# Streampunk/phaneron

Measured on AMD Instinct MI355X. Metric: frames/sec, 4-layer 2160p50 composite pipeline (v210 unpack->CSC->combine->CSC->v210 pack), higher is better.
Workload: dtype f32

## Files before the change

phaneron_amd/csrc/ph_api.cpp:

```cpp
#include <algorithm>
#include <atomic>
#include <chrono>
#include <cstdarg>
#include <cstdio>
#include <cstring>
#include <dlfcn.h>
#include <map>
#include <mutex>
#include <string>
#include <vector>

#include "../../include/phaneron_hip.h"
#include "ph_fused_field.h"
#include "ph_internal.h"
#include "ph_kernels.h"
#include "ph_lut_host.h"

using ph::KernelId;
using namespace ph;

namespace {
thread_local std::string g_err;
}

// ... 792 lines not shown
    ctx->luts.erase(it);
  }
  if (blob) {
    for (int q = 0; q < 3; ++q) hipStreamSynchronize(ctx->streams[q]);
    hipFree(blob);
  }
  return PH_OK;
}

int ph_lut_register(ph_ctx *ctx, const void *dev, const float *host) {
  if (!ctx || !dev || !host) return fail(PH_E_INVALID, "ph_lut_register: NULL argument");
  int rc = set_device(ctx);
  if (rc) return rc;
  ph_lut_unregister(ctx, dev);
  std::vector<uint32_t> blob;
  ph::LutHostInfo info;
  LutEntry e;
  if (ph::lut_compress(host, ph::kLutMaxLdsBytes, blob, info)) {
    if (!ctx->lds_base_checked.load()) {
      uint32_t *probe = nullptr, base = ~0u;
      PH_HIP(hipMalloc(&probe, 4));
      hipError_t pe = ph::launch_lds_base_probe(ctx->streams[0], probe);
      if (pe == hipSuccess) pe = hipStreamSynchronize(ctx->streams[0]);
      if (pe == hipSuccess) pe = hipMemcpy(&base, probe, 4, hipMemcpyDeviceToHost);
      hipFree(probe);
      if (pe != hipSuccess) return fail(PH_E_HIP, "ph_lut_register: LDS base probe: %s", hipGetErrorString(pe));
      if (base != 0) return fail(PH_E_HIP, "ph_lut_register: dynamic shared memory starts at LDS address %u, not 0: the table kernels cannot run", base);
      ctx->lds_base_checked.store(true);
    }
    const size_t blob_bytes = blob.size() * sizeof(uint32_t);
    PH_HIP(hipMalloc(&e.blob_dev, blob_bytes));
    PH_HIP(hipMemcpy(e.blob_dev, blob.data(), blob_bytes, hipMemcpyHostToDevice));
    e.view = ph::lut_view(info, e.blob_dev);
  }
  {
    std::lock_guard<std::mutex> lock(ctx->mu);
    ctx->luts[dev] = e;
  }
  return e.view.bytes ? 1 : 0;
}

int ph_lut_layout_of(const float *host, ph_lut_layout *layout, void *lds_image, size_t capacity) {
  if (!host || !layout) return fail(PH_E_INVALID, "ph_lut_layout_of: NULL argument");
  std::vector<uint32_t> blob;
  ph::LutHostInfo info;
  memset(layout, 0, sizeof(*layout));
  if (!ph::lut_compress(host, ph::kLutMaxLdsBytes, blob, info)) return 0;
  const ph::LutView v = ph::lut_view(info, nullptr);
  layout->lds_bytes = info.bytes, layout->hole = info.hole, layout->delta_off = info.delta_off, layout->shift = info.shift;
  layout->index_bias = (uint32_t)info.bias, layout->a_scale = v.a_scale;
  if (lds_image) {
    if (capacity < info.bytes) return fail(PH_E_INVALID, "ph_lut_layout_of: the image needs %u bytes, %zu given", info.bytes, capacity);
    memset(lds_image, 0, info.hole);
    memcpy(static_cast<char *>(lds_image) + info.hole, blob.data(), info.bytes - info.hole);
  }
  return (int)info.bytes;
}

int ph_debug_fused_lut_k(const float *host, uint32_t k5[5]) {
  if (!host || !k5) return fail(PH_E_INVALID, "ph_debug_fused_lut_k: NULL argument");
  std::vector<uint32_t> blob;
  ph::LutHostInfo info;
  if (!ph::lut_compress(host, ph::kLutMaxLdsBytes, blob, info)) return 0;
  const ph::FusedLutK k = ph::fused_lut_k(ph::lut_view(info, nullptr));
  memcpy(k5, &k, 5 * sizeof(uint32_t));
  return (int)info.bytes;
}
uint32_t ph_debug_fused_job_of(uint32_t wg_per_job, uint32_t block) {
  return wg_per_job ? ph::fused_job_of(block, ph::fused_wg_magic(wg_per_job)) : 0;
}
int ph_debug_fused_field_quad(uint32_t width, uint32_t height, int interlace, uint32_t g, uint32_t *f, uint32_t *line, uint32_t *col) {
  if (!width || width % 48) return fail(PH_E_INVALID, "ph_debug_fused_field_quad: width %u (the field launches take width %% 48 == 0)", width);
  if (interlace != 1 && interlace != 3) return fail(PH_E_INVALID, "ph_debug_fused_field_quad: interlace %d (a field: 1 or 3)", interlace);
  const uint32_t qpl = width / 6;
  if ((uint64_t)qpl * height * qpl >= (1ull << 32)) return fail(PH_E_INVALID, "ph_debug_fused_field_quad: %u x %u is beyond the kernels' division by reciprocal", width, height);
  if (g >= qpl * (height / 2u)) return fail(PH_E_INVALID, "ph_debug_fused_field_quad: quad %u is outside the field (%u quads)", g, qpl * (height / 2u));
  const ph::FieldQuad q = ph::fused_field_quad(g, qpl, (uint32_t)(((1ull << 32) + qpl - 1) / qpl), interlace == 3 ? 1u : 0u);
  if (f) *f = q.f;
  if (line) *line = q.line;
  if (col) *col = q.col;
  return PH_OK;
}
int ph_debug_image_nt(ph_ctx *ctx, size_t bytes) {
  if (!ctx) return fail(PH_E_INVALID, "ph_debug_image_nt: ctx is NULL");
  if (int rc = set_device(ctx)) return rc;
  return (int)ph::image_nt(bytes);
}

int ph_lut_query(ph_ctx *ctx, const void *dev, uint32_t *lds_bytes, uint32_t *toe, uint32_t *shift) {
  if (!ctx) return fail(PH_E_INVALID, "ph_lut_query: ctx is NULL");
  std::lock_guard<std::mutex> lock(ctx->mu);
  auto it = ctx->luts.find(dev);
  const bool have = it != ctx->luts.end();
  if (lds_bytes) *lds_bytes = have ? it->second.view.bytes : 0;
  if (toe) *toe = have ? (uint32_t)it->second.view.bias : 0;
  if (shift) *shift = have ? 23 - it->second.view.shift : 0;
  return PH_OK;
}

int ph_ctx_set_option(ph_ctx *ctx, const char *name, int value) {
// ... 29 lines not shown
    if (value != 0 && value != 1) return fail(PH_E_INVALID, "fused_multi_batch: 0 (a launch per such job) or 1 (shared launches)");
    return ctx->fused_multi_batch = value, PH_OK;
  }
  if (0 == strcmp(name, "fused_fields")) {
    if (value != 0 && value != 1) return fail(PH_E_INVALID, "fused_fields: 0 (the plain-layer launches compose the whole frame) or 1 (only the field, where every output takes the same one)");
    return ctx->fused_fields = value, PH_OK;
  }
  if (0 == strcmp(name, "host_pool_mb")) {
    if (value < 0) return fail(PH_E_INVALID, "host_pool_mb: a size in MiB");
    std::vector<ph_ctx::HostBlock> drop;
    {
      std::lock_guard<std::mutex> lock(ctx->mu);
      ctx->host_pool_mb = value;
      ctx->host_peak_bytes = ctx->host_live_bytes;
      while (ctx->host_pooled_bytes > (size_t)value << 20 && !ctx->host_pool.empty()) {
        auto it = std::prev(ctx->host_pool.end());
        ctx->host_pooled_bytes -= it->first;
        drop.push_back(it->second);
        ctx->host_pool.erase(it);
      }
    }
    for (auto &v : drop) {
      hipHostFree(v.p);
      if (v.busy) hipEventDestroy(v.busy);
    }
    return PH_OK;
  }
  return fail(PH_E_INVALID, "unknown option '%s'", name);
}

struct LutRef {
  ph::LutView view{};
  bool found = false;
  const ph::LutView *get() const { return found ? &view : nullptr; }
};
static LutRef lds_view(ph_ctx *ctx, const void *dev) {
  LutRef r;
  if (!ctx || !ctx->use_lds_lut) return r;
  std::lock_guard<std::mutex> lock(ctx->mu);
  auto it = ctx->luts.find(dev);
  if (it == ctx->luts.end() || !it->second.view.bytes) return r;
  r.view = it->second.view, r.found = true;
  return r;
}

extern "C++" void refresh_buf_lut(ph_ctx *ctx, ph_buf *b) {
  if (b->lut_dirty && b->hptr && b->bytes >= 65536 * 4) {
    hipStreamSynchronize(ctx->streams[PH_QUEUE_LOAD]);
    ph_lut_register(ctx, b->dptr, (const float *)b->hptr);
    b->lut_dirty = false;
  }
}

extern "C++" int chan_out_refused(const char *fn, int fmt) {
  return fail(PH_E_INVALID, "%s: the channel kernel does not write %s frames - run the separate kernels: the channel's frame as an image, then the format's writer (ph_pack_write)", fn,
              fmt_name(fmt));
}

extern "C++" bool inject_failure(ph_ctx *ctx) {
  const int v = ctx->fail_launches.load();
  if (v > 0) return true;
  if (v < 0 && ctx->fail_launches.fetch_add(1) == -1) ctx->fail_launches.store(1);
  return false;
}

uint32_t ph_v210_pitch_bytes(uint32_t width) { return width ? ph::v210_pitch_bytes(width) : 0; }

#define PH_LAUNCH(expr)                                                                         \
  do {                                                                                          \
    if (!ctx) return fail(PH_E_INVALID, "%s: ctx is NULL", __func__);                           \
    PH_QUEUE(__func__, queue);                                                                  \
    int rc_ = set_device(ctx);                                                                  \
    if (rc_) return rc_;                                                                        \
    hipError_t e_ = ph::trace_launch(#expr) ? hipSuccess : (expr);                              \
    if (e_ != hipSuccess) return fail(PH_E_HIP, "%s: launch failed: %s", __func__, hipGetErrorString(e_)); \
// ... 44 lines not shown
      PH_LAUNCH(ph::launch_v210_write_lds(stream_of(ctx, queue), in, out, width, height, interlace, cm, *v,
                                          (uint32_t)ctx->props.multiProcessorCount));
  }
  PH_LAUNCH(ph::launch_v210_write(stream_of(ctx, queue), in, out, width, height, interlace, cm, lut));
}

int ph_fused_v210_combine(ph_ctx *ctx, int queue, int n, const void *const *layers, void *out, uint32_t width,
                          uint32_t height, const void *rd_cm, const void *rd_lut, const void *rd_gm,
                          const void *wr_cm, const void *wr_lut) {
  if (n < 1 || n > ph::kMaxLayers) return fail(PH_E_INVALID, "ph_fused_v210_combine: 1..%d layers", ph::kMaxLayers);
  if (!layers || !out || !rd_cm || !rd_lut || !rd_gm || !wr_cm || !wr_lut || !width)
    return fail(PH_E_INVALID, "ph_fused_v210_combine: NULL/zero argument");
  const bool ragged = width % 48 != 0;
  if (width & 1) return fail(PH_E_INVALID, "ph_fused_v210_combine: width %u is odd; run the separate kernels", width);
  if (!height) return PH_OK;
  ph::FusedArgs a{};
  for (int i = 0; i < n; ++i) {
    if (!layers[i]) return fail(PH_E_INVALID, "ph_fused_v210_combine: layer %d is NULL", i);
    a.layers[i] = layers[i];
  }
  a.out = out;
  a.quads_per_line_used = width / 6;
  a.quads_per_line_pitch = ph::v210_pitch_bytes(width) / 16;
  a.total_quads = (ragged ? a.quads_per_line_pitch : a.quads_per_line_used) * height;
  a.tail_px = width % 6, a.magic_qpp = (uint32_t)(((1ull << 32) + a.quads_per_line_pitch - 1) / a.quads_per_line_pitch);
  if (ragged && (uint64_t)a.total_quads * a.quads_per_line_pitch >= (1ull << 32))
    return fail(PH_E_INVALID, "ph_fused_v210_combine: a %u x %u frame with ragged lines is too large; run the separate kernels", width, height);
  a.rd_cm = (const float *)rd_cm, a.rd_lut = (const float *)rd_lut, a.rd_gm = (const float *)rd_gm;
  a.wr_cm = (const float *)wr_cm, a.wr_lut = (const float *)wr_lut;
  if (ctx) {
    const LutRef rref = lds_view(ctx, rd_lut), wref = lds_view(ctx, wr_lut);
    const ph::LutView *rv = rref.get(), *wv = wref.get();
    if (rv && wv) {
      const ph::FusedLdsArgs la = ph::fused_lds_args(a, *rv, *wv);
      PH_LAUNCH(ph::launch_fused_v210_combine_lds(stream_of(ctx, queue), n, la, (uint32_t)ctx->props.multiProcessorCount));
    }
  }
  PH_LAUNCH(ph::launch_fused_v210_combine(stream_of(ctx, queue), n, a));
}

int ph_pack_plane_bytes(int format, uint32_t width, uint32_t height, size_t bytes[3]) {
  if (!bytes || !width) return fail(PH_E_INVALID, "ph_pack_plane_bytes: NULL/zero argument");
  if (const int rc = even_dims("ph_pack_plane_bytes", format, width, height)) return rc;
  const int n = ph::pack_plane_bytes(format, width, height, bytes);
  return n < 0 ? fail(PH_E_INVALID, "ph_pack_plane_bytes: unknown format %d", format) : n;
}

int ph_fused_v210_combine_batch(ph_ctx *ctx, int queue, int jobs, int n, const void *const *layers, void *const *outs,
                                uint32_t width, uint32_t height, const void *rd_cm, const void *rd_lut, const void *rd_gm,
                                const void *wr_cm, const void *wr_lut) {
  if (jobs < 1 || jobs > ph::kMaxBatch) return fail(PH_E_INVALID, "ph_fused_v210_combine_batch: 1..%d jobs", ph::kMaxBatch);
  if (n < 1 || n > ph::kMaxLayers) return fail(PH_E_INVALID, "ph_fused_v210_combine_batch: 1..%d layers", ph::kMaxLayers);
  if (!layers || !outs || !rd_cm || !rd_lut || !rd_gm || !wr_cm || !wr_lut)
    return fail(PH_E_INVALID, "ph_fused_v210_combine_batch: NULL argument");
  for (int j = 0; j < jobs; ++j) {
    if (!outs[j]) return fail(PH_E_INVALID, "ph_fused_v210_combine_batch: output %d is NULL", j);
    for (int l = 0; l < n; ++l)
      if (!layers[j * n + l]) return fail(PH_E_INVALID, "ph_fused_v210_combine_batch: job %d layer %d is NULL", j, l);
  }
  const LutRef rref = lds_view(ctx, rd_lut), wref = lds_view(ctx, wr_lut);
  const ph::LutView *rv = rref.get(), *wv = wref.get();
  if (jobs == 1 || !rv || !wv || !width || width % 48 || !height) {
    for (int j = 0; j < jobs; ++j) {
      int rc = ph_fused_v210_combine(ctx, queue, n, layers + (size_t)j * n, outs[j], width, height, rd_cm, rd_lut, rd_gm,
                                     wr_cm, wr_lut);
      if (rc != PH_OK) return rc;
    }
    return PH_OK;
  }
  ph::FusedArgs f{};
  for (int l = 0; l < n; ++l) f.layers[l] = layers[l];
  f.out = outs[0];
  f.quads_per_line_used = width / 6;
  f.quads_per_line_pitch = ph::v210_pitch_bytes(width) / 16;
  f.total_quads = f.quads_per_line_used * height;
  f.rd_cm = (const float *)rd_cm, f.rd_lut = (const float *)rd_lut, f.rd_gm = (const float *)rd_gm;
  f.wr_cm = (const float *)wr_cm, f.wr_lut = (const float *)wr_lut;
  ph::FusedLdsArgs la = ph::fused_lds_args(f, *rv, *wv);
  la.jobs = (uint32_t)jobs;
  for (int j = 1; j < jobs; ++j) {
    for (int l = 0; l < n; ++l) la.more_layers[j - 1][l] = layers[(size_t)j * n + l];
    la.more_out[j - 1] = outs[j];
  }
  PH_LAUNCH(ph::launch_fused_v210_combine_lds(stream_of(ctx, queue), n, la, (uint32_t)ctx->props.multiProcessorCount));
}

int ph_pack_read(ph_ctx *ctx, int queue, int format, const void *const planes[3], void *out, uint32_t width,
                 uint32_t height, const void *cm, const void *lut, const void *gm) {
  if (!ctx || !planes || !out || !lut || !gm || !width) return fail(PH_E_INVALID, "ph_pack_read: NULL/zero argument");
  if (format == PH_FMT_V210) return ph_v210_read(ctx, queue, planes[0], out, width, height, cm, lut, gm);
  if (const int rc = even_dims("ph_pack_read", format, width, height)) return rc;
  size_t pb[3];
  const int np = ph::pack_plane_bytes(format, width, height, pb);
  if (np < 0) return fail(PH_E_INVALID, "ph_pack_read: unknown format %d", format);
  for (int i = 0; i < np; ++i)
    if (!planes[i]) return fail(PH_E_INVALID, "ph_pack_read: plane %d is NULL", i);
  if (!fmt_rgb8(format) && !cm) return fail(PH_E_INVALID, "ph_pack_read: YCbCr formats need a colMatrix");
  if (!height) return PH_OK;
  PH_LAUNCH(ph::launch_pack_read(stream_of(ctx, queue), format, planes, out, width, height, cm, lut, gm, lds_view(ctx, lut).get(),
                                 (uint32_t)ctx->props.multiProcessorCount));
}

int ph_pack_read_batch(ph_ctx *ctx, int queue, int format, int n, const void *const (*planes)[3], void *const *outs, uint32_t width, uint32_t height,
                       const void *cm, const void *lut, const void *gm) {
  if (!ctx || !planes || !outs || !lut || !gm || !width) return fail(PH_E_INVALID, "ph_pack_read_batch: NULL/zero argument");
  if (n < 1 || n > ph::kMaxLayers) return fail(PH_E_INVALID, "ph_pack_read_batch: 1..%d frames", ph::kMaxLayers);
  if (const int rc = even_dims("ph_pack_read_batch", format, width, height)) return rc;
  const LutRef lref = lds_view(ctx, lut);
  const ph::LutView *v = format == PH_FMT_V210 ? nullptr : lref.get();
  if (n == 1 || !v) {
    if (format == PH_FMT_V210) {
// ... 2126 lines not shown
```

phaneron_amd/csrc/ph_internal.h:

```cpp
#pragma once
#include <atomic>
#include <cstdlib>
#include <map>
#include <mutex>
#include <string>
#include <vector>

#include "../../include/phaneron_hip.h"
#include "ph_kernels.h"
#include "ph_program.h"
#include "ph_spans.h"

static_assert(ph::kSpanLayers == ph::kMaxLayers && ph::kSpanOuts >= ph::kMaxChanOuts && ph::kSpanOuts >= ph::kMaxFusedOuts && ph::kSpanOuts >= ph::kMaxUpOuts,
              "a Footprint holds any job's ranges: ph_spans.h sizes it by these limits without seeing ph_kernels.h");
static_assert(ph::kMaxChanOps <= ph::kSpanLayers * 3, "a channel job's op list is at most three sources per layer");

#pragma GCC visibility push(hidden)
int fail(int code, const char *fmt, ...) __attribute__((format(printf, 2, 3)));
#pragma GCC visibility pop

#define PH_HIP(call)                                                                          \
  do {                                                                                        \
    hipError_t e_ = (call);                                                                   \
    if (e_ != hipSuccess) return fail(PH_E_HIP, "%s failed: %s", #call, hipGetErrorString(e_)); \
  } while (0)

struct LutEntry {
  ph::LutView view{};
  void *blob_dev = nullptr;
};

struct ph_ctx {
  int device = 0;
  std::map<const void *, LutEntry> luts;
  bool use_lds_lut = true;
  int stream_images = 0;
  int stream_threshold_mb = 64;
  hipStream_t streams[3] = {nullptr, nullptr, nullptr};
  hipDeviceProp_t props;
  std::multimap<size_t, void *> pool;
  size_t pooled_bytes = 0, live_buffers = 0, live_bytes = 0;
  struct HostBlock {
    void *p;
    hipEvent_t busy;
    uint64_t seq;
  };
  std::multimap<size_t, HostBlock> host_pool;
  size_t host_pooled_bytes = 0;
  uint64_t host_pool_seq = 0;
  int chan_enlarged = !(getenv("PH_CHAN_ENLARGED") && getenv("PH_CHAN_ENLARGED")[0] == '0');
  int chan_batch_outs = 0;
  int clip_batch = 0;
  int up_v210_tails = 0;
  int fused_multi_wgs = 0;
  int fused_multi_batch = 0;
  int fused_fields = 0;
  std::atomic<int> fail_launches{0};
  int host_pool_mb = 4096;
  size_t host_live_bytes = 0, host_peak_bytes = 0;
  uint64_t host_pins = 0;
  void *chan_index[3] = {nullptr, nullptr, nullptr};
  size_t chan_index_bytes[3] = {0, 0, 0};
// ... 62 lines not shown
```

phaneron_amd/csrc/ph_kernels.h:

```cpp
#pragma once
#include <hip/hip_runtime.h>
#include <stddef.h>
#include <stdint.h>

#include "ph_formats.h"
#include "ph_lut.h"

namespace ph {

constexpr int kMaxLayers = 8;
constexpr int kMaxDynamicLds = 160 * 1024;

extern thread_local uint32_t t_stream_images;
extern thread_local uint32_t t_stream_threshold_mb;
static inline uint32_t image_nt(size_t bytes) {
  return t_stream_images == 2 ? (bytes > ((size_t)t_stream_threshold_mb << 20) ? 1u : 0u) : t_stream_images;
}

struct FusedArgs {
  const void *layers[kMaxLayers];
  void *out;
  uint32_t quads_per_line_used;
  uint32_t quads_per_line_pitch;
  uint32_t total_quads;
// ... 4 lines not shown
constexpr int kMaxBatch = 8;
struct FusedLutK {
  float a_scale, a_base, delta_scale, delta_base;
  uint32_t a_shift;
};
FusedLutK fused_lut_k(const LutView &v);

static inline uint32_t fused_wg_magic(uint32_t wg_per_job) { return (uint32_t)(((1ull << 31) + wg_per_job - 1) / wg_per_job); }
static inline __host__ __device__ uint32_t fused_job_of(uint32_t block, uint32_t magic) {
#if defined(__HIP_DEVICE_COMPILE__)
  return __umulhi(2u * block + 1u, magic);
#else
  return (uint32_t)(((uint64_t)(2u * block + 1u) * magic) >> 32);
#endif
}

struct alignas(64) FusedLdsArgs {
  const uint32_t *rd_blob;
  uint32_t rd_bytes, rd_hole;
  uint32_t total_quads;
  uint32_t wg_per_job;
  uint32_t per_wg;
  uint32_t magic_wg;
  const void *layers[kMaxLayers];
  void *out;
  const float *rd_cm, *rd_gm, *wr_cm;
  FusedLutK rd_k, wr_k;
  uint32_t wr_bytes, wr_hole;
  const uint32_t *wr_blob;
  uint32_t jobs;
  uint32_t quads_per_line_used;
  uint32_t quads_per_line_pitch;
  uint32_t tail_px, magic_qpp;
  const void *more_layers[kMaxBatch - 1][kMaxLayers];
  void *more_out[kMaxBatch - 1];
};
constexpr size_t kFusedHeadBytes = 192;
static_assert(offsetof(FusedLdsArgs, rd_blob) == 0 && offsetof(FusedLdsArgs, rd_bytes) == 8 && offsetof(FusedLdsArgs, rd_hole) == 12 &&
              offsetof(FusedLdsArgs, total_quads) == 16 && offsetof(FusedLdsArgs, wg_per_job) == 20 && offsetof(FusedLdsArgs, per_wg) == 24 &&
              offsetof(FusedLdsArgs, magic_wg) == 28 && offsetof(FusedLdsArgs, layers) == 32,
              "line 0 of the fused kernel's head: ph_kernels_lds.hip reads it by offset");
static_assert(offsetof(FusedLdsArgs, out) == 96 && offsetof(FusedLdsArgs, rd_cm) == 104 && offsetof(FusedLdsArgs, rd_gm) == 112 &&
              offsetof(FusedLdsArgs, wr_cm) == 120, "the head's pointers end with the first 128 bytes");
static_assert(offsetof(FusedLdsArgs, rd_k) == 128 && offsetof(FusedLdsArgs, wr_k) == 148 && offsetof(FusedLdsArgs, wr_bytes) == 168 &&
              offsetof(FusedLdsArgs, wr_hole) == 172 && offsetof(FusedLdsArgs, wr_blob) == 176 && offsetof(FusedLdsArgs, jobs) == 184 &&
              offsetof(FusedLdsArgs, quads_per_line_used) == 188 && offsetof(FusedLdsArgs, quads_per_line_pitch) == kFusedHeadBytes,
              "line 2 of the fused kernel's head");
static_assert(offsetof(FusedLdsArgs, more_layers) >= kFusedHeadBytes, "the batch arrays lie behind the head");
FusedLdsArgs fused_lds_args(const FusedArgs &f, const LutView &rd, const LutView &wr);

constexpr int kMaxFusedOuts = 4;
struct FusedOut {
  uint32_t fmt;
  uint32_t takes;
  uint32_t line_end;
  uint32_t field;
  uint32_t half_pitch;
  uint32_t pad;
  const float *wr_cm;
  void *plane[3];
  LutView wr;
};
struct FusedMultiArgs {
  const void *layers[kMaxLayers];
  uint32_t quads_per_line, total_quads;
  uint32_t magic_qpl, need_line;
  const float *rd_cm, *rd_gm;
  LutView rd;
  uint32_t n_out;
  FusedOut out[kMaxFusedOuts];
};
hipError_t launch_fused_v210_combine_multi(hipStream_t s, int n, const FusedMultiArgs &a, uint32_t num_cus, uint32_t max_wgs);
hipError_t fused_multi_plan(const FusedMultiArgs &a, uint32_t num_cus, uint32_t max_wgs, FusedMultiArgs &b, uint32_t &grid, uint32_t &lds);
struct FusedMultiBatchArgs {
  FusedMultiArgs m;
  const void *layers[kMaxBatch][kMaxLayers];
  void *plane[kMaxBatch][kMaxFusedOuts][3];
};
hipError_t launch_fused_v210_combine_multi_batch(hipStream_t s, int n, uint32_t jobs, const FusedMultiBatchArgs &a, uint32_t num_cus, uint32_t max_wgs);
enum : uint32_t { kFusedCut = 0, kFusedDissolve = 1, kFusedWipeV210 = 2, kFusedWipeF32 = 3 };
struct FusedTransArgs {
  FusedMultiArgs m;
// ... 356 lines not shown
```

phaneron_amd/csrc/ph_kernels_lds.hip:

```cpp
#include "ph_device.h"
#include "ph_kernels.h"
#include "ph_ldslut.h"

#include <atomic>
#include <cstdlib>

#include <type_traits>
#include <utility>

#pragma clang fp contract(off)

#ifndef PH_PROBE
#define PH_PROBE 0
#endif
#if PH_PROBE
constexpr int kProbeWords = 16;
__device__ unsigned long long g_fused_probe[2048 * kProbeWords];
extern "C" int ph_debug_fused_probe(unsigned long long *out, int n_words) {
  return (int)hipMemcpyFromSymbol(out, HIP_SYMBOL(g_fused_probe), (size_t)n_words * 8);
}
#define PH_STAMP_ENTRY() \
  const unsigned long long ph_entry_cycles = __builtin_amdgcn_s_memtime(), ph_entry_ticks = __builtin_amdgcn_s_memrealtime()
#define PH_STAMP(k) PH_STAMP_IF(k, tile_begin == wg_begin)
#define PH_STAMP_IF(k, first_tile)                                                   \
// ... 78 lines not shown
  k.g = make_float4(cm[4], cm[5], cm[6], cm[7]);
  k.b = make_float4(cm[8], cm[9], cm[10], cm[11]);
#pragma unroll
  for (int i = 0; i < 9; ++i) k.gm[i] = gm[i];
  return k;
}
__device__ __forceinline__ WriteK load_write_k(const_f32_ptr cm) {
  WriteK k;
  k.y = make_float4(cm[0], cm[1], cm[2], cm[3]);
  k.u = make_float4(cm[4], cm[5], cm[6], cm[7]);
  k.v = make_float4(cm[8], cm[9], cm[10], cm[11]);
  return k;
}
static_assert(kFusedHeadBytes == 3 * sizeof(fused_head_line), "fused_head_load asks for three lines");
__device__ __forceinline__ FusedHead fused_head_load() {
  FusedHead h;
  const auto *args = __builtin_amdgcn_kernarg_segment_ptr();
  asm volatile("s_load_dwordx16 %0, %3, 0x0\n\ts_load_dwordx16 %1, %3, 0x40\n\ts_load_dwordx16 %2, %3, 0x80\n\ts_waitcnt lgkmcnt(0)"
               : "=&s"(h.l0), "=&s"(h.l1), "=&s"(h.l2)
               : "s"(args));
  return h;
}

constexpr int kLayerFirst = 1, kLayerLast = 2;
template <int... I, typename F>
__device__ __forceinline__ void static_for_each(std::integer_sequence<int, I...>, F &&f) {
  (f(std::integral_constant<int, I>{}), ...);
}
template <int COUNT, typename F>
__device__ __forceinline__ void static_for(F &&f) {
  static_for_each(std::make_integer_sequence<int, COUNT>{}, f);
}
template <int PLACE, bool STD>
__device__ __forceinline__ void fused_layer_combine(float (&acc)[18], const uint4 w, const ReadK &rk, const LutK &rlut, float last) {
  __builtin_amdgcn_sched_barrier(0);
  const Yuv6 q = unpack_quad(w);
#pragma unroll
  for (int j = 0; j < 6; ++j) {
    const float4 t = read_px_lds<STD>(q.y[j], q.cb[j >> 1], q.cr[j >> 1], rk, rlut, last);
    if (PLACE & kLayerFirst) {
      acc[3 * j] = t.x, acc[3 * j + 1] = t.y, acc[3 * j + 2] = t.z;
      if (PLACE & kLayerLast) {
#pragma unroll
        for (int c = 0; c < 3; ++c) acc[3 * j + c] = __builtin_fminf(__builtin_fmaxf(acc[3 * j + c], 0.0f), 1.0f);
      }
      asm volatile("" : "+v"(acc[3 * j]), "+v"(acc[3 * j + 1]), "+v"(acc[3 * j + 2]));
    } else {
      const float kk = 1.0f - t.w;
      if (PLACE & kLayerLast)
        asm volatile("v_fma_f32 %0, %0, %3, %4 clamp\n\tv_fma_f32 %1, %1, %3, %5 clamp\n\tv_fma_f32 %2, %2, %3, %6 clamp"
                     : "+v"(acc[3 * j]), "+v"(acc[3 * j + 1]), "+v"(acc[3 * j + 2])
                     : "v"(kk), "v"(t.x), "v"(t.y), "v"(t.z));
      else
        asm volatile("v_fma_f32 %0, %0, %3, %4\n\tv_fma_f32 %1, %1, %3, %5\n\tv_fma_f32 %2, %2, %3, %6"
                     : "+v"(acc[3 * j]), "+v"(acc[3 * j + 1]), "+v"(acc[3 * j + 2])
                     : "v"(kk), "v"(t.x), "v"(t.y), "v"(t.z));
    }
  }
}
__device__ __forceinline__ float lds_lut_index_clamped(float t) { return t * 65535.0f + kRoundMagic; }
__device__ __forceinline__ float lds_lut_index_clamped_tail(float t, bool trunc) {
  const float x = t * 65535.0f;
  return (trunc ? __builtin_floorf(x) : x) + kRoundMagic;
}

template <int N, int P, int BS, bool PIPE = false, int MODE = 0, bool TAIL = false>
__global__ __launch_bounds__(BS) void fused_v210_combine_lds_kernel(FusedLdsArgs a, uint32_t *handoff = nullptr) {
  static_assert(!TAIL || (!PIPE && MODE == 0), "the tail instantiation exists for the shipped form only");
  PH_STAMP_ENTRY();
  FusedHead head = fused_head_load();
  const uint32_t total_quads = head.word(offsetof(FusedLdsArgs, total_quads)), wg_per_job = head.word(offsetof(FusedLdsArgs, wg_per_job));
  const uint32_t per_wg = head.word(offsetof(FusedLdsArgs, per_wg));
  uint32_t job = fused_job_of(blockIdx.x, head.word(offsetof(FusedLdsArgs, magic_wg)));
  asm("" : "+s"(job));
  const uint32_t wg_in_job = blockIdx.x - job * wg_per_job;
  auto layer_ptr = [&](int l) { return reinterpret_cast<const uint4 *>(job ? a.more_layers[job - 1][l] : a.layers[l]); };
  const uint32_t wg_begin = wg_in_job * per_wg;
  const uint32_t wg_end = wg_begin + per_wg < total_quads ? wg_begin + per_wg : total_quads;
  if (wg_begin >= wg_end) return;
  const uint32_t tile_quads = BS * P;
  auto quad_at = [&](uint32_t tile_begin, int p) {
    const uint32_t f = tile_begin + p * BS + threadIdx.x;
    return f < wg_end ? f : wg_end - 1;
  };
  constexpr bool kSplitLayers = !PIPE && MODE == 0;
  if (kSplitLayers && job) {
    auto own_layer = [&](int l) {
      const uintptr_t p = (uintptr_t)a.more_layers[job - 1][l];
      head.set_word(offsetof(FusedLdsArgs, layers) + 8 * l, (uint32_t)p);
// ... 8 lines not shown
    if (N > 6) own_layer(6);
    if (N > 7) own_layer(7);
  }
  static_assert(N <= 8, "the layers' pointers are named one by one");
  typedef const __attribute__((address_space(1))) char *global_byte_ptr;
  auto layer_base = [&](int l) { return (global_byte_ptr)head.ptr<global_quad_ptr>(offsetof(FusedLdsArgs, layers) + 8 * l); };
  auto layer_word = [&](int l, uint32_t at) { return load_stream((global_quad_ptr)(layer_base(l) + at)); };
  auto layer_word_any = [&](int l, uint32_t at) {
    global_byte_ptr base = layer_base(N - 1);
    if (N > 3 && l == 2) base = layer_base(2);
    if (N > 4 && l == 3) base = layer_base(3);
    if (N > 5 && l == 4) base = layer_base(4);
    if (N > 6 && l == 5) base = layer_base(5);
    if (N > 7 && l == 6) base = layer_base(6);
    return load_stream((global_quad_ptr)(base + at));
  };
  uint4 w;
  if (kSplitLayers) w = layer_word(0, quad_at(wg_begin, 0) << 4);
  else if (job) w = load_stream(layer_ptr(0) + quad_at(wg_begin, 0));
  else w = load_stream(head.ptr<global_quad_ptr>(offsetof(FusedLdsArgs, layers)) + quad_at(wg_begin, 0));
  const uint32_t *const rd_blob = (const uint32_t *)head.ptr<global_u32_ptr>(offsetof(FusedLdsArgs, rd_blob));
  const uint32_t rd_bytes = head.word(offsetof(FusedLdsArgs, rd_bytes)), rd_hole = head.word(offsetof(FusedLdsArgs, rd_hole));
  PH_STAMP_IF(0, true);
  if (MODE != 2) lds_lut_load<BS, false>(rd_blob, rd_bytes, rd_hole);
  __builtin_amdgcn_sched_barrier(0);
  const ReadK rk = load_read_k(head.ptr<const_f32_ptr>(offsetof(FusedLdsArgs, rd_cm)), head.ptr<const_f32_ptr>(offsetof(FusedLdsArgs, rd_gm)));
  const WriteK wk = load_write_k(head.ptr<const_f32_ptr>(offsetof(FusedLdsArgs, wr_cm)));
  LutK rlut = head.lut_k(offsetof(FusedLdsArgs, rd_k)), wlut = head.lut_k(offsetof(FusedLdsArgs, wr_k));
  asm("" : "+v"(rlut.a_base), "+v"(rlut.delta_base), "+v"(wlut.a_base), "+v"(wlut.delta_base));
  const uint32_t *const wr_blob = (const uint32_t *)head.ptr<global_u32_ptr>(offsetof(FusedLdsArgs, wr_blob));
  const uint32_t wr_bytes = head.word(offsetof(FusedLdsArgs, wr_bytes)), wr_hole = head.word(offsetof(FusedLdsArgs, wr_hole));
  uint4 *const out_ptr = reinterpret_cast<uint4 *>(job ? a.more_out[job - 1] : a.out);
  const bool std_matrix = ycbcr_matrix_is_standard(rk);
  for (uint32_t tile_begin = wg_begin; tile_begin < wg_end; tile_begin += tile_quads) {
    uint32_t st[P][9];
    auto quad_of = [&](int p) { return quad_at(tile_begin, p); };
    if (tile_begin != wg_begin) {
      w = kSplitLayers ? layer_word(0, quad_of(0) << 4) : load_stream(layer_ptr(0) + quad_of(0));
      if (MODE == 0) lds_lut_load<BS, false>(rd_blob, rd_bytes, rd_hole);
    }
    auto slot_kind = [&](uint32_t f) -> uint32_t {
      const uint32_t g = f - __umulhi(f, a.magic_qpp) * a.quads_per_line_pitch;
      return g < a.quads_per_line_used ? 0u : (g == a.quads_per_line_used && a.tail_px) ? 1u : 2u;
    };
    auto phase1_slice = [&](auto tag, uint4 w, uint32_t f, uint32_t f_next, bool more, uint32_t(&st)[9]) -> uint4 {
      const bool in_tail = TAIL && slot_kind(f) == 1u;
      const float last = TAIL ? (in_tail ? 0.0f : 1.0f) : 1.0f;
      float acc[18];
#pragma unroll
      for (int i = 0; i < 18; ++i) acc[i] = 0.0f;
#pragma unroll 1
      for (int l = 0; l < N; ++l) {
        uint4 nxt = w;
        if (l + 1 < N) nxt = load_stream(layer_ptr(l + 1) + f);
        else if (more) nxt = load_stream(layer_ptr(0) + f_next);
        const Yuv6 q = unpack_quad(w);
#pragma unroll
        for (int j = 0; j < 6; ++j) {
          const float4 t = read_px_lds<decltype(tag)::value>(q.y[j], q.cb[j >> 1], q.cr[j >> 1], rk, rlut, last);
          const float kk = 1.0f - t.w;
          asm volatile("v_fma_f32 %0, %0, %3, %4\n\tv_fma_f32 %1, %1, %3, %5\n\tv_fma_f32 %2, %2, %3, %6"
                       : "+v"(acc[3 * j]), "+v"(acc[3 * j + 1]), "+v"(acc[3 * j + 2])
                       : "v"(kk), "v"(t.x), "v"(t.y), "v"(t.z));
        }
        w = nxt;
      }
#pragma unroll
      for (int i = 0; i < 9; ++i) {
        const uint32_t lo = __float_as_uint(TAIL ? lds_lut_index_unit_tail(acc[2 * i], in_tail) : lds_lut_index_unit(acc[2 * i]));
        const uint32_t hi = __float_as_uint(TAIL ? lds_lut_index_unit_tail(acc[2 * i + 1], in_tail) : lds_lut_index_unit(acc[2 * i + 1]));
        st[i] = __builtin_amdgcn_perm(hi, lo, 0x05040100u);
        asm volatile("" : "+v"(st[i]));
      }
      return w;
    };
    auto phase1_slice_split = [&](auto tag, uint4 w, uint32_t f, uint32_t f_next, bool more, uint32_t(&st)[9]) __attribute__((always_inline)) -> uint4 {
      constexpr int MID = N > 2 ? N - 2 : 0;
      const bool in_tail = TAIL && slot_kind(f) == 1u;
      const float last = TAIL ? (in_tail ? 0.0f : 1.0f) : 1.0f;
      float acc[18];
      constexpr bool STD = decltype(tag)::value;
      auto combine = [&](auto place, const uint4 word) __attribute__((always_inline)) {
        fused_layer_combine<decltype(place)::value, STD>(acc, word, rk, rlut, last);
      };
      constexpr std::integral_constant<int, N == 1 ? (kLayerFirst | kLayerLast) : kLayerFirst> first_layer{};
      constexpr std::integral_constant<int, 0> middle_layer{};
      constexpr std::integral_constant<int, kLayerLast> last_layer{};
      uint32_t at = f << 4;
      if (STD) asm volatile("; standard matrix" : "+v"(at));
      else asm volatile("; any matrix" : "+v"(at));
      uint4 nxt = w;
      if (N > 1) nxt = layer_word(1, at);
      else if (more) nxt = layer_word(0, f_next << 4);
      combine(first_layer, w);
      w = nxt;
      if constexpr (MID > 0 && MID <= 2) {
        nxt = layer_word(2, at);
        combine(middle_layer, w);
        w = nxt;
        if constexpr (MID == 2) {
          nxt = layer_word(3, at);
          combine(middle_layer, w);
          w = nxt;
        }
      } else if constexpr (MID > 2) {
#pragma unroll 1
        for (int l = 1; l + 1 <= MID; l += 2) {
          const uint4 w2 = layer_word_any(l + 1, at);
          combine(middle_layer, w);
          w = layer_word_any(l + 2, at);
          combine(middle_layer, w2);
        }
        if (MID & 1) {
          nxt = layer_word(N - 1, at);
          combine(middle_layer, w);
          w = nxt;
// ... 98 lines not shown
          PH_BALANCE(p);
          const uint32_t f = tile_begin + p * BS + threadIdx.x;
          uint32_t y[6], u[3], v[3];
#pragma unroll
          for (int j = 0; j < 6; ++j) {
            PxPending nx = wp;
            if (j < 5) nx = write_px_issue(idx_at(p, 3 * j + 3), idx_at(p, 3 * j + 4), idx_at(p, 3 * j + 5), wlut);
            else if (p + 1 < P) {
              if ((p + 1) * BS < tile_left) nx = write_px_issue(idx_at(p + 1 < P ? p + 1 : p, 0), idx_at(p + 1 < P ? p + 1 : p, 1), idx_at(p + 1 < P ? p + 1 : p, 2), wlut);
            }
            __builtin_amdgcn_sched_barrier(0);
            const float gr = lds_lut_finish(wp.r), gg = lds_lut_finish(wp.g), gb = lds_lut_finish(wp.b);
            y[j] = sat_u16_rte(dot4(gr, gg, gb, 1.0f, wk.y));
            if ((j & 1) == 0) {
              u[j >> 1] = sat_u16_rte(dot4(gr, gg, gb, 1.0f, wk.u));
              v[j >> 1] = sat_u16_rte(dot4(gr, gg, gb, 1.0f, wk.v));
            }
            __builtin_amdgcn_sched_barrier(0);
            wp = nx;
          }
          if (f < wg_end) store_stream(out_ptr + f, pack_quad(y, u, v));
        }
      }
    } else {
    const uint32_t wave_first = (uint32_t)__builtin_amdgcn_readfirstlane((int)(threadIdx.x & ~63u));
    if constexpr (kSplitLayers) {
      static_for<P>([&](auto slice) __attribute__((always_inline)) {
        constexpr int p = decltype(slice)::value;
        const uint32_t f = quad_of(p);
        if (p * BS + wave_first < wg_end - tile_begin) {
          PH_BALANCE(p);
          const bool more = (p + 1 < P) && ((p + 1) * BS + wave_first < wg_end - tile_begin);
          const uint32_t f_next = more ? quad_of(p + 1) : f;
          if (std_matrix) w = phase1_slice_split(std::true_type{}, w, f, f_next, more, st[p]);
          else w = phase1_slice_split(std::false_type{}, w, f, f_next, more, st[p]);
        }
      });
    } else if (MODE != 2) {
#pragma unroll
    for (int p = 0; p < P; ++p) {
      const uint32_t f = quad_of(p);
      if (p * BS + wave_first < wg_end - tile_begin) {
        PH_BALANCE(p);
        const bool more = (p + 1 < P) && ((p + 1) * BS + wave_first < wg_end - tile_begin);
        const uint32_t f_next = more ? quad_of(p + 1) : f;
        if (std_matrix) w = phase1_slice(std::true_type{}, w, f, f_next, more, st[p]);
        else w = phase1_slice(std::false_type{}, w, f, f_next, more, st[p]);
      }
    }
    }
    if (MODE == 1) {
#pragma unroll
      for (int p = 0; p < P; ++p)
        if (p * BS + wave_first < wg_end - tile_begin) {
          const uint32_t f = quad_of(p);
#pragma unroll
          for (int i = 0; i < 9; ++i) handoff[(size_t)i * a.total_quads + f] = st[p][i];
        }
      continue;
    }
    if (MODE == 2) {
#pragma unroll
      for (int p = 0; p < P; ++p)
        if (p * BS + wave_first < wg_end - tile_begin) {
          const uint32_t f = quad_of(p);
#pragma unroll
          for (int i = 0; i < 9; ++i) st[p][i] = __builtin_nontemporal_load(handoff + (size_t)i * a.total_quads + f);
        }
// ... 519 lines not shown
}

template <typename K>
static hipError_t allow_lds(K kernel, uint32_t bytes) {
  return hipFuncSetAttribute(reinterpret_cast<const void *>(kernel), hipFuncAttributeMaxDynamicSharedMemorySize, kMaxDynamicLds);
}
template <typename K>
static hipError_t allow_lds_once(K kernel, std::atomic<uint64_t> &done) {
  int dev = 0;
  hipError_t e = hipGetDevice(&dev);
  if (e != hipSuccess) return e;
  const uint64_t bit = 1ull << (dev & 63);
  if (dev < 64 && (done.load(std::memory_order_acquire) & bit)) return hipSuccess;
  e = allow_lds(kernel, kMaxDynamicLds);
  if (e == hipSuccess && dev < 64) done.fetch_or(bit, std::memory_order_release);
  return e;
}

FusedLutK fused_lut_k(const LutView &v) {
#if defined(__x86_64__)
  const unsigned csr = __builtin_ia32_stmxcsr();
  __builtin_ia32_ldmxcsr(csr & ~0x8040u);
#endif
  const volatile float lds0 = 0.0f, magic = 12582912.0f;
  const float small = (v.delta_base + lds0) + v.bias * v.delta_scale;
  const float b = small - magic * v.delta_scale;
  const FusedLutK k{v.a_scale, -((magic - v.bias) * v.a_scale), v.delta_scale, b, v.shift - 2u};
#if defined(__x86_64__)
  __builtin_ia32_ldmxcsr(csr);
#endif
  return k;
}

FusedLdsArgs fused_lds_args(const FusedArgs &f, const LutView &rd, const LutView &wr) {
  FusedLdsArgs a{};
  a.rd_blob = rd.blob, a.rd_bytes = rd.bytes, a.rd_hole = rd.hole;
  a.wr_blob = wr.blob, a.wr_bytes = wr.bytes, a.wr_hole = wr.hole;
  a.rd_k = fused_lut_k(rd), a.wr_k = fused_lut_k(wr);
  for (int l = 0; l < kMaxLayers; ++l) a.layers[l] = f.layers[l];
  a.out = f.out, a.rd_cm = f.rd_cm, a.rd_gm = f.rd_gm, a.wr_cm = f.wr_cm;
  a.total_quads = f.total_quads, a.quads_per_line_used = f.quads_per_line_used, a.quads_per_line_pitch = f.quads_per_line_pitch;
  a.tail_px = f.tail_px, a.magic_qpp = f.magic_qpp, a.jobs = 1;
  return a;
}

#if PH_FUSED_SPLIT
template <int N, int P, int BS, int MODE>
static hipError_t launch_fused_half(hipStream_t s, FusedLdsArgs b, uint32_t lds) {
  static uint32_t *handoff = nullptr;
  static size_t handoff_quads = 0;
  if (handoff_quads < b.total_quads) {
    if (handoff) hipFree(handoff);
    if (hipMalloc(&handoff, (size_t)b.total_quads * 36) != hipSuccess) return hipErrorOutOfMemory;
    handoff_quads = b.total_quads;
  }
  static std::atomic<uint64_t> lds_allowed{0};
  hipError_t e = allow_lds_once(fused_v210_combine_lds_kernel<N, P, BS, false, MODE>, lds_allowed);
  if (e != hipSuccess) return e;
  fused_v210_combine_lds_kernel<N, P, BS, false, MODE><<<b.wg_per_job * b.jobs, BS, lds, s>>>(b, handoff);
  return hipGetLastError();
}
#endif

template <int N, int P, int BS, bool PIPE = false, bool TAIL = false>
static hipError_t launch_fused_npb(hipStream_t s, const FusedLdsArgs &a, uint32_t grid_in, uint32_t lds) {
  uint32_t grid = grid_in;
#if PH_FUSED_SPLIT
  static const int cus_env = [] {
// ... 169 lines not shown
```

phaneron_amd/csrc/ph_ldslut.h:

```cpp
#pragma once
#include "ph_device.h"
#include "ph_lut.h"

#pragma clang fp contract(off)

namespace ph {

constexpr int kLdsBlock = 1024;

#ifndef PH_ABLATE
#define PH_ABLATE 0
#endif

extern __shared__ __attribute__((aligned(16))) unsigned char g_lds[];

template <int BS = kLdsBlock, bool WAIT = true>
__device__ __forceinline__ void lds_lut_load(const uint32_t *blob, uint32_t bytes, uint32_t hole) {
#if PH_ABLATE & 2
  return;
#endif
  const uint32_t n = (bytes - hole) / 16;
  unsigned char *const dst = g_lds + hole;
  const uint32_t wave = threadIdx.x >> 6, lane = threadIdx.x & 63;
  const uint4 *src = reinterpret_cast<const uint4 *>(blob);
// ... 114 lines not shown
  for (int j = 0; j < 4; ++j) {
    const float gr = lds_lut_fetch(lut, yi[3 * j]), gg = lds_lut_fetch(lut, yi[3 * j + 1]);
    const float gb = lds_lut_fetch(lut, yi[3 * j + 2]);
    y[j] = sat_u16_trunc(__builtin_roundf(dot4(gr, gg, gb, 1.0f, wk.y)));
    if ((j & 1) == 0) {
      u[j >> 1] = sat_u16_trunc(__builtin_roundf(dot4(gr, gg, gb, 1.0f, wk.u)));
      v[j >> 1] = sat_u16_trunc(__builtin_roundf(dot4(gr, gg, gb, 1.0f, wk.v)));
    }
  }
  uint4 w = make_uint4(v[0] << 20 | y[0] << 10 | u[0], 0u, 0u, 0u);
  if (remain == 2u) {
    w.y = y[1];
  } else if (remain == 4u) {
    w.y = y[2] << 20 | u[1] << 10 | y[1];
    w.z = y[3] << 10 | v[1];
  }
  return w;
}

struct LutInLds {
  LutK k;
  __device__ __forceinline__ float at(float x) const { return lds_lut_at(k, x); }
  __device__ __forceinline__ float at_unit(float t) const { return lds_lut_at_unit(k, t); }
};
struct LutInGlobal {
  const float *__restrict__ t;
  __device__ __forceinline__ float at(float x) const { return t[sat_u16_rte(x)]; }
  __device__ __forceinline__ float at_unit(float u) const { return t[sat_u16_rte(u * 65535.0f)]; }
};

__device__ __forceinline__ bool ycbcr_matrix_is_standard(const ReadK &k) {
  return k.r.y == 0.0f && k.b.z == 0.0f && k.r.x == k.g.x && k.g.x == k.b.x;
}
template <bool STD = false>
__device__ __forceinline__ float4 read_px_lds(float y, float cb, float cr, const ReadK &k, const LutK &lut, float last = 1.0f) {
  float tr, tg, tb;
  if (STD) {
    const float ym = y * k.r.x;
    tr = fma_rn(last, k.r.w, fma_rn(cr, k.r.z, ym));
    tg = fma_rn(last, k.g.w, fma_rn(cr, k.g.z, fma_rn(cb, k.g.y, ym)));
    tb = fma_rn(last, k.b.w, fma_rn(cb, k.b.y, ym));
  } else {
    tr = dot4(y, cb, cr, last, k.r), tg = dot4(y, cb, cr, last, k.g), tb = dot4(y, cb, cr, last, k.b);
  }
  const float r = lds_lut_at_unit(lut, tr);
  const float g = lds_lut_at_unit(lut, tg);
  const float b = lds_lut_at_unit(lut, tb);
  return make_float4(dot3(r, g, b, k.gm[0], k.gm[1], k.gm[2]), dot3(r, g, b, k.gm[3], k.gm[4], k.gm[5]),
                     dot3(r, g, b, k.gm[6], k.gm[7], k.gm[8]), 1.0f);
}

struct PxPending {
  LutPending r, g, b;
};
template <bool STD>
__device__ __forceinline__ PxPending read_px_issue(float y, float cb, float cr, const ReadK &k, const LutK &lut, float last = 1.0f) {
  float tr, tg, tb;
  if (STD) {
    const float ym = y * k.r.x;
    tr = fma_rn(last, k.r.w, fma_rn(cr, k.r.z, ym));
    tg = fma_rn(last, k.g.w, fma_rn(cr, k.g.z, fma_rn(cb, k.g.y, ym)));
    tb = fma_rn(last, k.b.w, fma_rn(cb, k.b.y, ym));
  } else {
    tr = dot4(y, cb, cr, last, k.r), tg = dot4(y, cb, cr, last, k.g), tb = dot4(y, cb, cr, last, k.b);
  }
  PxPending p;
// ... 35 lines not shown
```

phaneron_amd/csrc/ph_lut.cpp:

```cpp
#include "ph_lut_host.h"

#include <algorithm>
#include <cmath>
#include <cstring>

namespace ph {

namespace {
inline uint32_t f2u(float f) {
  uint32_t u;
  std::memcpy(&u, &f, 4);
  return u;
}
inline float u2f(uint32_t u) {
  float f;
  std::memcpy(&f, &u, 4);
  return f;
}
}

LutView lut_view(const LutHostInfo &info, const void *blob_dev) {
  LutView v;
  v.blob = static_cast<const uint32_t *>(blob_dev);
  v.bytes = info.bytes;
  v.hole = info.hole;
  v.bias = info.bias;
  v.shift = info.shift;
  v.a_scale = std::ldexp(1.0f, 1 - (int)(f2u(info.bias) >> 23));
  v.delta_scale = u2f(2u);
  v.delta_base = u2f(info.delta_off - 2u * (uint32_t)info.bias);
  return v;
}

bool lut_compress(const float *lut, uint32_t max_bytes, std::vector<uint32_t> &blob, LutHostInfo &info) {
  std::vector<uint32_t> p(65536), blk(65536);
  std::memcpy(p.data(), lut, 65536 * sizeof(uint32_t));
  bool found = false;
  for (float bias : {16.0f, 32.0f, 64.0f, 128.0f}) {
    for (uint32_t m = 7; m <= 10; ++m) {
      const uint32_t shift = 23 - m;
      const uint32_t first = f2u(bias) >> shift;
      const uint32_t n_blocks = (f2u(65535.0f + bias) >> shift) - first + 1;
      const uint32_t n_anchors = (n_blocks + 3) & ~3u;
      const uint32_t hole = 4u << m;
      const uint32_t bytes = hole + n_anchors * 4 + 65536 * 2;
      if (bytes > max_bytes || (found && bytes >= info.bytes)) continue;
      std::vector<uint32_t> lo(n_blocks, 0xffffffffu), hi(n_blocks, 0);
      for (uint32_t i = 0; i < 65536; ++i) {
        blk[i] = (f2u((float)i + bias) >> shift) - first;
        lo[blk[i]] = std::min(lo[blk[i]], p[i]);
        hi[blk[i]] = std::max(hi[blk[i]], p[i]);
      }
      bool ok = true;
      for (uint32_t b = 0; b < n_blocks && ok; ++b)
        if (lo[b] != 0xffffffffu && hi[b] - lo[b] >= 65536u) ok = false;
      if (!ok) continue;
      found = true;
      info.bytes = bytes, info.shift = shift, info.first = first, info.n_anchors = n_anchors;
      info.hole = hole, info.delta_off = hole + n_anchors * 4, info.bias = bias;
      blob.assign((bytes - hole) / 4, 0);
      for (uint32_t b = 0; b < n_blocks; ++b) blob[b] = lo[b] == 0xffffffffu ? 0 : lo[b];
      uint16_t *delta = reinterpret_cast<uint16_t *>(blob.data() + n_anchors);
      for (uint32_t i = 0; i < 65536; ++i) delta[i] = (uint16_t)(p[i] - lo[blk[i]]);
    }
// ... 27 lines not shown
```

phaneron_amd/csrc/ph_lut_host.h:

```cpp
#pragma once
#include <stdint.h>
#include <vector>

#include "ph_lut.h"

namespace ph {

struct LutHostInfo {
  uint32_t bytes = 0, shift = 0, first = 0, n_anchors = 0, delta_off = 0, hole = 0;
  float bias = 0;
};

constexpr uint32_t kLutMaxLdsBytes = 160 * 1024;

bool lut_compress(const float *lut65536, uint32_t max_bytes, std::vector<uint32_t> &blob, LutHostInfo &info);
LutView lut_view(const LutHostInfo &info, const void *blob_dev);

}
```

Before: 20800.

## Replace opaque-layer blend with a zero-weighted witness chain and last-layer clamp

Since v210 layers carry no alpha, every layer is opaque and the composite equals the top layer. Lower layers now only feed a zero-weighted witness accumulator, kept so NaN and Inf still propagate as before. The top layer's colour is written with a clamp. This drops the alpha path and the per-channel blend FMAs from the combine loop. A host-side bound on the largest finite value of the read LUT, passed in a spare kernel-argument slot, proves the zero-multiply chain cannot overflow; when the bound fails the kernel falls back to the older non-split slice path.

```diff
diff --git a/phaneron_amd/csrc/ph_api.cpp b/phaneron_amd/csrc/ph_api.cpp
--- a/phaneron_amd/csrc/ph_api.cpp
+++ b/phaneron_amd/csrc/ph_api.cpp
@@ -848,6 +848,7 @@
     PH_HIP(hipMalloc(&e.blob_dev, blob_bytes));
     PH_HIP(hipMemcpy(e.blob_dev, blob.data(), blob_bytes, hipMemcpyHostToDevice));
     e.view = ph::lut_view(info, e.blob_dev);
+    e.max_finite = ph::lut_max_finite(host);
   }
   {
     std::lock_guard<std::mutex> lock(ctx->mu);
@@ -882,6 +883,13 @@
   memcpy(k5, &k, 5 * sizeof(uint32_t));
   return (int)info.bytes;
 }
+int ph_debug_fused_witness(const float *host, const float *gm9, float *lmax, int *holds) {
+  if (!host || !gm9 || !lmax || !holds) return fail(PH_E_INVALID, "ph_debug_fused_witness: NULL argument");
+  const ph::FusedLdsArgs a = ph::fused_lds_args(ph::FusedArgs{}, ph::LutView{}, ph::LutView{}, ph::lut_max_finite(host));
+  *lmax = a.rd_lmax;
+  *holds = ph::fused_witness_holds(a.rd_lmax, gm9) ? 1 : 0;
+  return PH_OK;
+}
 uint32_t ph_debug_fused_job_of(uint32_t wg_per_job, uint32_t block) {
   return wg_per_job ? ph::fused_job_of(block, ph::fused_wg_magic(wg_per_job)) : 0;
 }
@@ -977,6 +985,7 @@
 struct LutRef {
   ph::LutView view{};
   bool found = false;
+  float max_finite = __builtin_inff();
   const ph::LutView *get() const { return found ? &view : nullptr; }
 };
 static LutRef lds_view(ph_ctx *ctx, const void *dev) {
@@ -985,7 +994,7 @@
   std::lock_guard<std::mutex> lock(ctx->mu);
   auto it = ctx->luts.find(dev);
   if (it == ctx->luts.end() || !it->second.view.bytes) return r;
-  r.view = it->second.view, r.found = true;
+  r.view = it->second.view, r.max_finite = it->second.max_finite, r.found = true;
   return r;
 }
 
@@ -1096,7 +1105,7 @@
     const LutRef rref = lds_view(ctx, rd_lut), wref = lds_view(ctx, wr_lut);
     const ph::LutView *rv = rref.get(), *wv = wref.get();
     if (rv && wv) {
-      const ph::FusedLdsArgs la = ph::fused_lds_args(a, *rv, *wv);
+      const ph::FusedLdsArgs la = ph::fused_lds_args(a, *rv, *wv, rref.max_finite);
       PH_LAUNCH(ph::launch_fused_v210_combine_lds(stream_of(ctx, queue), n, la, (uint32_t)ctx->props.multiProcessorCount));
     }
   }
@@ -1140,7 +1149,7 @@
   f.total_quads = f.quads_per_line_used * height;
   f.rd_cm = (const float *)rd_cm, f.rd_lut = (const float *)rd_lut, f.rd_gm = (const float *)rd_gm;
   f.wr_cm = (const float *)wr_cm, f.wr_lut = (const float *)wr_lut;
-  ph::FusedLdsArgs la = ph::fused_lds_args(f, *rv, *wv);
+  ph::FusedLdsArgs la = ph::fused_lds_args(f, *rv, *wv, rref.max_finite);
   la.jobs = (uint32_t)jobs;
   for (int j = 1; j < jobs; ++j) {
     for (int l = 0; l < n; ++l) la.more_layers[j - 1][l] = layers[(size_t)j * n + l];
diff --git a/phaneron_amd/csrc/ph_internal.h b/phaneron_amd/csrc/ph_internal.h
--- a/phaneron_amd/csrc/ph_internal.h
+++ b/phaneron_amd/csrc/ph_internal.h
@@ -28,6 +28,7 @@
 struct LutEntry {
   ph::LutView view{};
   void *blob_dev = nullptr;
+  float max_finite = __builtin_inff();
 };
 
 struct ph_ctx {
diff --git a/phaneron_amd/csrc/ph_kernels.h b/phaneron_amd/csrc/ph_kernels.h
--- a/phaneron_amd/csrc/ph_kernels.h
+++ b/phaneron_amd/csrc/ph_kernels.h
@@ -60,6 +60,7 @@
   uint32_t quads_per_line_used;
   uint32_t quads_per_line_pitch;
   uint32_t tail_px, magic_qpp;
+  float rd_lmax;
   const void *more_layers[kMaxBatch - 1][kMaxLayers];
   void *more_out[kMaxBatch - 1];
 };
@@ -75,7 +76,17 @@
               offsetof(FusedLdsArgs, quads_per_line_used) == 188 && offsetof(FusedLdsArgs, quads_per_line_pitch) == kFusedHeadBytes,
               "line 2 of the fused kernel's head");
 static_assert(offsetof(FusedLdsArgs, more_layers) >= kFusedHeadBytes, "the batch arrays lie behind the head");
-FusedLdsArgs fused_lds_args(const FusedArgs &f, const LutView &rd, const LutView &wr);
+static inline __host__ __device__ bool fused_witness_holds(float lmax, const float *gm) {
+  const float bound = 8.5070591730234616e37f, half = 4.2535295865117308e37f;
+  bool ok = lmax < half;
+  for (int i = 0; i < 3; ++i) {
+    const float row = (__builtin_fabsf(gm[3 * i]) + __builtin_fabsf(gm[3 * i + 1])) + __builtin_fabsf(gm[3 * i + 2]);
+    ok = ok & (lmax * row < bound);
+  }
+  return ok;
+}
+static_assert(offsetof(FusedLdsArgs, rd_lmax) == 204 && offsetof(FusedLdsArgs, more_layers) == 208, "rd_lmax fills a gap behind the head: no other field moves");
+FusedLdsArgs fused_lds_args(const FusedArgs &f, const LutView &rd, const LutView &wr, float rd_lmax);
 
 constexpr int kMaxFusedOuts = 4;
 struct FusedOut {
diff --git a/phaneron_amd/csrc/ph_kernels_lds.hip b/phaneron_amd/csrc/ph_kernels_lds.hip
--- a/phaneron_amd/csrc/ph_kernels_lds.hip
+++ b/phaneron_amd/csrc/ph_kernels_lds.hip
@@ -134,29 +134,28 @@
   static_for_each(std::make_integer_sequence<int, COUNT>{}, f);
 }
 template <int PLACE, bool STD>
-__device__ __forceinline__ void fused_layer_combine(float (&acc)[18], const uint4 w, const ReadK &rk, const LutK &rlut, float last) {
+__device__ __forceinline__ void fused_layer_combine(float (&acc)[18], float (&wit)[6], const uint4 w, const ReadK &rk, const LutK &rlut, float last) {
   __builtin_amdgcn_sched_barrier(0);
   const Yuv6 q = unpack_quad(w);
 #pragma unroll
   for (int j = 0; j < 6; ++j) {
-    const float4 t = read_px_lds<STD>(q.y[j], q.cb[j >> 1], q.cr[j >> 1], rk, rlut, last);
-    if (PLACE & kLayerFirst) {
-      acc[3 * j] = t.x, acc[3 * j + 1] = t.y, acc[3 * j + 2] = t.z;
-      if (PLACE & kLayerLast) {
-#pragma unroll
-        for (int c = 0; c < 3; ++c) acc[3 * j + c] = __builtin_fminf(__builtin_fmaxf(acc[3 * j + c], 0.0f), 1.0f);
-      }
+    if constexpr (PLACE == (kLayerFirst | kLayerLast)) {
+      const float4 t = read_px_lds<STD>(q.y[j], q.cb[j >> 1], q.cr[j >> 1], rk, rlut, last);
+      acc[3 * j] = __builtin_fminf(__builtin_fmaxf(t.x, 0.0f), 1.0f);
+      acc[3 * j + 1] = __builtin_fminf(__builtin_fmaxf(t.y, 0.0f), 1.0f);
+      acc[3 * j + 2] = __builtin_fminf(__builtin_fmaxf(t.z, 0.0f), 1.0f);
       asm volatile("" : "+v"(acc[3 * j]), "+v"(acc[3 * j + 1]), "+v"(acc[3 * j + 2]));
+    } else if constexpr (PLACE == kLayerLast) {
+      const float4 t = read_px_lds<STD>(q.y[j], q.cb[j >> 1], q.cr[j >> 1], rk, rlut, last);
+      asm volatile("v_fma_f32 %0, %1, 0, %2 clamp" : "=v"(acc[3 * j]) : "v"(wit[j]), "v"(t.x));
+      asm volatile("v_fma_f32 %0, %1, 0, %2 clamp" : "=v"(acc[3 * j + 1]) : "v"(wit[j]), "v"(t.y));
+      asm volatile("v_fma_f32 %0, %1, 0, %2 clamp" : "=v"(acc[3 * j + 2]) : "v"(wit[j]), "v"(t.z));
     } else {
-      const float kk = 1.0f - t.w;
-      if (PLACE & kLayerLast)
-        asm volatile("v_fma_f32 %0, %0, %3, %4 clamp\n\tv_fma_f32 %1, %1, %3, %5 clamp\n\tv_fma_f32 %2, %2, %3, %6 clamp"
-                     : "+v"(acc[3 * j]), "+v"(acc[3 * j + 1]), "+v"(acc[3 * j + 2])
-                     : "v"(kk), "v"(t.x), "v"(t.y), "v"(t.z));
+      const Rgb1 e = read_px_lds_rgb<STD>(q.y[j], q.cb[j >> 1], q.cr[j >> 1], rk, rlut, last);
+      if constexpr (PLACE == kLayerFirst)
+        asm volatile("v_mul_f32 %0, 0, %1\n\tv_fma_f32 %0, %2, 0, %0\n\tv_fma_f32 %0, %3, 0, %0" : "=&v"(wit[j]) : "v"(e.r), "v"(e.g), "v"(e.b));
       else
-        asm volatile("v_fma_f32 %0, %0, %3, %4\n\tv_fma_f32 %1, %1, %3, %5\n\tv_fma_f32 %2, %2, %3, %6"
-                     : "+v"(acc[3 * j]), "+v"(acc[3 * j + 1]), "+v"(acc[3 * j + 2])
-                     : "v"(kk), "v"(t.x), "v"(t.y), "v"(t.z));
+        asm volatile("v_fma_f32 %0, %1, 0, %0\n\tv_fma_f32 %0, %2, 0, %0\n\tv_fma_f32 %0, %3, 0, %0" : "+v"(wit[j]) : "v"(e.r), "v"(e.g), "v"(e.b));
     }
   }
 }
@@ -231,6 +230,11 @@
   const uint32_t wr_bytes = head.word(offsetof(FusedLdsArgs, wr_bytes)), wr_hole = head.word(offsetof(FusedLdsArgs, wr_hole));
   uint4 *const out_ptr = reinterpret_cast<uint4 *>(job ? a.more_out[job - 1] : a.out);
   const bool std_matrix = ycbcr_matrix_is_standard(rk);
+  bool witness = false;
+  if (kSplitLayers && N > 1) {
+    const float rd_lmax = ((const_f32_ptr)__builtin_amdgcn_kernarg_segment_ptr())[offsetof(FusedLdsArgs, rd_lmax) / 4];
+    witness = fused_witness_holds(rd_lmax, rk.gm);
+  }
   for (uint32_t tile_begin = wg_begin; tile_begin < wg_end; tile_begin += tile_quads) {
     uint32_t st[P][9];
     auto quad_of = [&](int p) { return quad_at(tile_begin, p); };
@@ -242,7 +246,7 @@
       const uint32_t g = f - __umulhi(f, a.magic_qpp) * a.quads_per_line_pitch;
       return g < a.quads_per_line_used ? 0u : (g == a.quads_per_line_used && a.tail_px) ? 1u : 2u;
     };
-    auto phase1_slice = [&](auto tag, uint4 w, uint32_t f, uint32_t f_next, bool more, uint32_t(&st)[9]) -> uint4 {
+    auto phase1_slice = [&](auto tag, uint4 w, uint32_t f, uint32_t f_next, bool more, uint32_t(&st)[9]) __attribute__((always_inline)) -> uint4 {
       const bool in_tail = TAIL && slot_kind(f) == 1u;
       const float last = TAIL ? (in_tail ? 0.0f : 1.0f) : 1.0f;
       float acc[18];
@@ -277,10 +281,10 @@
       constexpr int MID = N > 2 ? N - 2 : 0;
       const bool in_tail = TAIL && slot_kind(f) == 1u;
       const float last = TAIL ? (in_tail ? 0.0f : 1.0f) : 1.0f;
-      float acc[18];
+      float acc[18], wit[6];
       constexpr bool STD = decltype(tag)::value;
       auto combine = [&](auto place, const uint4 word) __attribute__((always_inline)) {
-        fused_layer_combine<decltype(place)::value, STD>(acc, word, rk, rlut, last);
+        fused_layer_combine<decltype(place)::value, STD>(acc, wit, word, rk, rlut, last);
       };
       constexpr std::integral_constant<int, N == 1 ? (kLayerFirst | kLayerLast) : kLayerFirst> first_layer{};
       constexpr std::integral_constant<int, 0> middle_layer{};
@@ -445,8 +449,13 @@
           PH_BALANCE(p);
           const bool more = (p + 1 < P) && ((p + 1) * BS + wave_first < wg_end - tile_begin);
           const uint32_t f_next = more ? quad_of(p + 1) : f;
-          if (std_matrix) w = phase1_slice_split(std::true_type{}, w, f, f_next, more, st[p]);
-          else w = phase1_slice_split(std::false_type{}, w, f, f_next, more, st[p]);
+          if (N == 1 || witness) {
+            if (std_matrix) w = phase1_slice_split(std::true_type{}, w, f, f_next, more, st[p]);
+            else w = phase1_slice_split(std::false_type{}, w, f, f_next, more, st[p]);
+          } else {
+            if (std_matrix) w = phase1_slice(std::true_type{}, w, f, f_next, more, st[p]);
+            else w = phase1_slice(std::false_type{}, w, f, f_next, more, st[p]);
+          }
         }
       });
     } else if (MODE != 2) {
@@ -1032,8 +1041,9 @@
   return k;
 }
 
-FusedLdsArgs fused_lds_args(const FusedArgs &f, const LutView &rd, const LutView &wr) {
+FusedLdsArgs fused_lds_args(const FusedArgs &f, const LutView &rd, const LutView &wr, float rd_lmax) {
   FusedLdsArgs a{};
+  a.rd_lmax = rd_lmax;
   a.rd_blob = rd.blob, a.rd_bytes = rd.bytes, a.rd_hole = rd.hole;
   a.wr_blob = wr.blob, a.wr_bytes = wr.bytes, a.wr_hole = wr.hole;
   a.rd_k = fused_lut_k(rd), a.wr_k = fused_lut_k(wr);
diff --git a/phaneron_amd/csrc/ph_ldslut.h b/phaneron_amd/csrc/ph_ldslut.h
--- a/phaneron_amd/csrc/ph_ldslut.h
+++ b/phaneron_amd/csrc/ph_ldslut.h
@@ -170,6 +170,26 @@
 __device__ __forceinline__ bool ycbcr_matrix_is_standard(const ReadK &k) {
   return k.r.y == 0.0f && k.b.z == 0.0f && k.r.x == k.g.x && k.g.x == k.b.x;
 }
+struct Rgb1 {
+  float r, g, b;
+};
+template <bool STD = false>
+__device__ __forceinline__ Rgb1 read_px_lds_rgb(float y, float cb, float cr, const ReadK &k, const LutK &lut, float last = 1.0f) {
+  float tr, tg, tb;
+  if (STD) {
+    const float ym = y * k.r.x;
+    tr = fma_rn(last, k.r.w, fma_rn(cr, k.r.z, ym));
+    tg = fma_rn(last, k.g.w, fma_rn(cr, k.g.z, fma_rn(cb, k.g.y, ym)));
+    tb = fma_rn(last, k.b.w, fma_rn(cb, k.b.y, ym));
+  } else {
+    tr = dot4(y, cb, cr, last, k.r), tg = dot4(y, cb, cr, last, k.g), tb = dot4(y, cb, cr, last, k.b);
+  }
+  Rgb1 o;
+  o.r = lds_lut_at_unit(lut, tr);
+  o.g = lds_lut_at_unit(lut, tg);
+  o.b = lds_lut_at_unit(lut, tb);
+  return o;
+}
 template <bool STD = false>
 __device__ __forceinline__ float4 read_px_lds(float y, float cb, float cr, const ReadK &k, const LutK &lut, float last = 1.0f) {
   float tr, tg, tb;
diff --git a/phaneron_amd/csrc/ph_lut.cpp b/phaneron_amd/csrc/ph_lut.cpp
--- a/phaneron_amd/csrc/ph_lut.cpp
+++ b/phaneron_amd/csrc/ph_lut.cpp
@@ -30,6 +30,15 @@
   v.delta_scale = u2f(2u);
   v.delta_base = u2f(info.delta_off - 2u * (uint32_t)info.bias);
   return v;
+}
+
+float lut_max_finite(const float *lut) {
+  uint32_t top = 0;
+  for (int i = 0; i < 65536; ++i) {
+    const uint32_t mag = f2u(lut[i]) & 0x7FFFFFFFu;
+    if (mag < 0x7F800000u && mag > top) top = mag;
+  }
+  return u2f(top);
 }
 
 bool lut_compress(const float *lut, uint32_t max_bytes, std::vector<uint32_t> &blob, LutHostInfo &info) {
diff --git a/phaneron_amd/csrc/ph_lut_host.h b/phaneron_amd/csrc/ph_lut_host.h
--- a/phaneron_amd/csrc/ph_lut_host.h
+++ b/phaneron_amd/csrc/ph_lut_host.h
@@ -15,5 +15,6 @@
 
 bool lut_compress(const float *lut65536, uint32_t max_bytes, std::vector<uint32_t> &blob, LutHostInfo &info);
 LutView lut_view(const LutHostInfo &info, const void *blob_dev);
+float lut_max_finite(const float *lut65536);
 
 }
```

New measurement: 21040, median of 6. 1.1% higher.
